# pinellolab/GRAFIMO

Measured on AMD Instinct MI355X. Metric: scored haplotype k-mers/sec, higher is better.
Workload: dtype int32

## Files before the change

### grafimo_amd/csrc/gfm_score_quad.hpp

```cpp
#pragma once

#include "gfm_score_kernels.hpp"
#include "gfm_quad_launch.hpp"

namespace {

typedef unsigned u32x2_t __attribute__((ext_vector_type(2)));
typedef unsigned u32x4_t __attribute__((ext_vector_type(4)));
typedef __attribute__((address_space(3))) const u32x2_t lds_cu32x2;
typedef __attribute__((address_space(3))) const u32x4_t lds_cu32x4;
typedef int i32x4 __attribute__((ext_vector_type(4)));

template <int W, int MM, bool STORE = true>
__global__ void __launch_bounds__(kThreads)
score_quad_kernel(const uint8_t *__restrict__ kmers, long long n, long long row_base, const ScoreArgs<MM> a)
{
    extern __shared__ __attribute__((aligned(16))) unsigned char smem[];
    constexpr int NDW = (W + 3) / 4;
    constexpr int kTabBytes = quad_tab_bytes(W, MM);
    constexpr int CB = kQuadRows * W;
    constexpr int kLoads = (CB + 1023) / 1024;
    constexpr int GP = quad_pitch(W);
    constexpr int PAD = quad_pad(W);
    constexpr int SSTRIDE = quad_strip_stride(W, MM);

    if (lds_offset(smem) != 0u) __builtin_trap();
    const int tid = threadIdx.x;
    const int lane = tid & (kWave - 1);
    const int wave = __builtin_amdgcn_readfirstlane(tid >> 6);
    const int n_waves = (int)(blockDim.x >> 6);
    const int wg_threads = (int)blockDim.x;
    unsigned char *tab = smem;
    unsigned char *stage_base = smem + kTabBytes;
    unsigned *hist[MM];
    {
        unsigned *h = reinterpret_cast<unsigned *>(stage_base + n_waves * SSTRIDE);
#pragma unroll
        for (int m = 0; m < MM; ++m) {
            hist[m] = h;
            if (a.m[m].use_hist) h += a.m[m].nb + 1;
        }
    }

    unsigned char *stage = stage_base + wave * SSTRIDE;
    const unsigned stage_off = (unsigned)(kTabBytes + wave * SSTRIDE);
    const long long nfull = n / kQuadRows;
    const long long cstride = (long long)gridDim.x * n_waves;
    bool vec_store = true;
    const bool through = a.store_through == 1;
    constexpr bool no_store = !STORE;
#pragma unroll
    for (int m = 0; m < MM; ++m) vec_store = vec_store && (reinterpret_cast<uintptr_t>(a.m[m].scores) & 15u) == 0;

    uint4 pre[kQuadDepth][kLoads];
    auto fetch = [&](uint4 (&dst)[kLoads], long long c) {
        const uint8_t *src = kmers + c * (long long)CB + lane * 16;
#pragma unroll
        for (int i = 0; i < kLoads; ++i) {
            if (i * 1024 + 1024 <= CB || i * 1024 + lane * 16 < CB) {
                typedef unsigned u32x4 __attribute__((ext_vector_type(4)));
                const u32x4 t = __builtin_nontemporal_load(reinterpret_cast<const u32x4 *>(src + i * 1024));
                dst[i] = make_uint4(t.x, t.y, t.z, t.w);
            }
        }
    };

    long long *hitq[MM];
    int qn[MM];
    bool select[MM];
#pragma unroll
    for (int m = 0; m < MM; ++m) {
        hitq[m] = reinterpret_cast<long long *>(stage + quad_stage_bytes(W)) + m * kHitQueue;
        qn[m] = 0;
        select[m] = a.m[m].cutoff != GFM_NO_SELECT;
        if (select[m] && blockIdx.x == 0 && tid == 0)
            a.m[m].ctl->snap[a.m[m].slot] = a.m[m].hit_count ? *a.m[m].hit_count : 0ull;
    }

    int p_score[MM][4];
    long long p_crow = -1;
    auto book = [&]() {
        const int k0 = 4 * lane;
#pragma unroll
        for (int m = 0; m < MM; ++m) {
            const MotifArgs &ma = a.m[m];
            if (ma.use_hist) {
#pragma unroll
                for (int j = 0; j < 4; ++j) {
                    const unsigned off = (unsigned)(p_score[m][j] - ma.lo);
                    if (off < (unsigned)ma.nb)
                        atomicAdd(&hist[m][off], 1u);
                    else if (p_score[m][j] == ma.min_val)
                        atomicAdd(&hist[m][ma.nb], 1u);
                    else
                        atomicAdd(&ma.spill[(size_t)(blockIdx.x & (kSpillCopies - 1)) * (size_t)ma.spill_n + (size_t)(p_score[m][j] - ma.spill_lo)], 1u);
                }
            }
            if (select[m]) {
                const int best = max(max(p_score[m][0], p_score[m][1]), max(p_score[m][2], p_score[m][3]));
                if (__builtin_amdgcn_ballot_w64(best >= ma.cutoff)) {
#pragma unroll
                    for (int j = 0; j < 4; ++j)
                        hitq_push(hitq[m], qn[m], p_score[m][j] >= ma.cutoff,
                                  ((row_base + p_crow + k0 + j) << GFM_HIT_SCORE_BITS) | (long long)p_score[m][j], lane,
                                  ma.hit_count, &ma.ctl->mid[ma.slot], ma.hit_rows, ma.hit_cap);
                }
            }
        }
    };

    long long c = (long long)blockIdx.x * n_waves + wave;
#pragma unroll
    for (int d = 0; d < kQuadDepth; ++d)
        if (c + d * cstride < nfull) fetch(pre[d], c + d * cstride);
    if constexpr (MM == 1) {
        for (int i = tid; i < kTabBytes / 2; i += wg_threads) reinterpret_cast<uint16_t *>(tab)[i] = a.m[0].tab[i];
    } else {
        for (int i = tid; i < kTabBytes / 8; i += wg_threads) {
            unsigned long long v = 0;
            if (a.m[0].tab[i] == kPoison) {
                v = 1ull << 57;
            } else {
#pragma unroll
                for (int m = 0; m < MM; ++m) v |= (unsigned long long)a.m[m].tab[i] << (19 * m);
            }
            reinterpret_cast<unsigned long long *>(tab)[i] = v;
        }
    }
#pragma unroll
    for (int m = 0; m < MM; ++m)
        if (a.m[m].use_hist)
            for (int i = tid; i <= a.m[m].nb; i += wg_threads) hist[m][i] = 0u;
    __syncthreads();

    while (c < nfull) {
#pragma unroll
        for (int d = 0; d < kQuadDepth; ++d) {
            if (c >= nfull) break;
            const long long crow = c * kQuadRows;
            if (p_crow >= 0) book();
#pragma unroll
            for (int i = 0; i < kLoads; ++i) {
                const int off = i * 1024 + lane * 16;
                if (i * 1024 + 1024 <= CB || off < CB) {
                    const int dst = PAD ? off + PAD * (off / (4 * W)) : off;
                    *reinterpret_cast<uint4 *>(stage + dst) = pre[d][i];
                }
            }
            if (c + kQuadDepth * cstride < nfull) fetch(pre[d], c + kQuadDepth * cstride);
            __builtin_amdgcn_fence(__ATOMIC_RELEASE, "wavefront");
            __builtin_amdgcn_wave_barrier();

            unsigned w[W + 1];
            {
                const unsigned base = stage_off + (unsigned)(lane * GP);
                if constexpr (W % 2 == 1) {
#pragma unroll
                    for (int t = 0; t < W; ++t) w[t] = ((lds_cu32 *)(uintptr_t)base)[t];
                } else if constexpr (W % 4 == 2) {
#pragma unroll
                    for (int t = 0; t < W / 2; ++t) {
                        const u32x2_t v = ((lds_cu32x2 *)(uintptr_t)base)[t];
                        w[2 * t] = v.x;
                        w[2 * t + 1] = v.y;
                    }
                } else {
#pragma unroll
                    for (int t = 0; t < W / 4; ++t) {
                        const u32x4_t v = ((lds_cu32x4 *)(uintptr_t)base)[t];
                        w[4 * t] = v.x;
                        w[4 * t + 1] = v.y;
                        w[4 * t + 2] = v.z;
                        w[4 * t + 3] = v.w;
                    }
                }
                w[W] = 0u;
            }
            int score[MM][4];
#pragma unroll
            for (int j = 0; j < 4; ++j) {
                const int r = (j * W) & 3;
                bool any_n;
                int acc[MM];
                if constexpr (MM == 1) {
                    int s1 = 0;
#pragma unroll
                    for (int t = 0; t < NDW; ++t) {
                        const int q = (j * W + 4 * t) >> 2;
                        const unsigned x = r ? __builtin_amdgcn_alignbit(w[q + 1], w[q], (unsigned)(8 * r)) : w[q];
                        unsigned y;
                        asm("v_bfi_b32 %0, %1, %2, %3" : "=v"(y) : "s"(0x000E000Eu), "v"(x), "v"(x >> 5));
                        const unsigned e0 = y & 0x7Eu;
                        const unsigned e1 = (y >> 16) & 0x7Eu;
                        s1 += *(lds_cu16 *)(uintptr_t)(e0 + (unsigned)((2 * t) * 128));
                        s1 += *(lds_cu16 *)(uintptr_t)(e1 + (unsigned)((2 * t + 1) * 128));
                    }
                    any_n = (unsigned)s1 >= kPoison;
                    acc[0] = s1;
                } else {
                    unsigned long long s64 = 0;
#pragma unroll
                    for (int t = 0; t < NDW; ++t) {
                        const int q = (j * W + 4 * t) >> 2;
                        const unsigned x = r ? __builtin_amdgcn_alignbit(w[q + 1], w[q], (unsigned)(8 * r)) : w[q];
                        unsigned y;
                        asm("v_bfi_b32 %0, %1, %2, %3" : "=v"(y) : "s"(0x000E000Eu), "v"(x), "v"(x >> 5));
                        const unsigned e0 = (y & 0x7Eu) << 2;
                        const unsigned e1 = ((y >> 16) & 0x7Eu) << 2;
                        s64 += *(lds_cu64 *)(uintptr_t)(e0 + (unsigned)((2 * t) * 512));
                        s64 += *(lds_cu64 *)(uintptr_t)(e1 + (unsigned)((2 * t + 1) * 512));
                    }
                    any_n = (s64 >> 57) != 0;
#pragma unroll
                    for (int m = 0; m < MM; ++m) acc[m] = (int)((s64 >> (19 * m)) & 0x7FFFFull);
                }
#pragma unroll
                for (int m = 0; m < MM; ++m) score[m][j] = any_n ? a.m[m].min_val : acc[m];
            }
            const int k0 = 4 * lane;
#pragma unroll
            for (int m = 0; m < MM; ++m) {
                const __amdgpu_buffer_rsrc_t rs =
                    __builtin_amdgcn_make_buffer_rsrc(a.m[m].scores + crow, 0, kQuadRows * 4, 0x00020000);
                if (no_store) {
                } else if (vec_store) {
                    const u32x4_t out = {(unsigned)score[m][0], (unsigned)score[m][1], (unsigned)score[m][2],
                                         (unsigned)score[m][3]};
                    if (through)
                        __builtin_amdgcn_raw_buffer_store_b128(out, rs, k0 * 4, 0, kStoreThrough);
                    else
                        __builtin_amdgcn_raw_buffer_store_b128(out, rs, k0 * 4, 0, kStoreStream);
                } else {
#pragma unroll
                    for (int j = 0; j < 4; ++j) {
                        if (through)
                            __builtin_amdgcn_raw_buffer_store_b32((unsigned)score[m][j], rs, (k0 + j) * 4, 0, kStoreThrough);
                        else
                            __builtin_amdgcn_raw_buffer_store_b32((unsigned)score[m][j], rs, (k0 + j) * 4, 0, kStoreStream);
                    }
                }
#pragma unroll
                for (int j = 0; j < 4; ++j) p_score[m][j] = score[m][j];
            }
            p_crow = crow;
            __builtin_amdgcn_fence(__ATOMIC_ACQUIRE, "wavefront");
            __builtin_amdgcn_wave_barrier();
            c += cstride;
        }
    }
    if (p_crow >= 0) book();
    if (blockIdx.x == gridDim.x - 1 && wave == n_waves - 1 && nfull * kQuadRows < n) {
        const long long first = nfull * kQuadRows;
        const int count = (int)(n - first);
#pragma unroll 1
        for (int r0 = 0; r0 < count; r0 += kWave) {
            const int k = r0 + lane;
            const bool live = k < count;
            const uint8_t *row = kmers + (first + (live ? k : 0)) * (long long)W;
            unsigned long long s64 = 0;
            bool bad = false;
#pragma unroll 1
            for (int p = 0; p < 2 * NDW; ++p) {
                const unsigned b0 = 2 * p < W ? row[2 * p] : (unsigned)'A';
                const unsigned b1 = 2 * p + 1 < W ? row[2 * p + 1] : (unsigned)'A';
                const unsigned e = p * 64 + ((b0 >> 1) & 7u) + 8u * ((b1 >> 1) & 7u);
                if constexpr (MM == 1) {
                    const unsigned v = reinterpret_cast<const uint16_t *>(tab)[e];
                    bad = bad || v == kPoison;
                    s64 += v;
                } else {
                    s64 += reinterpret_cast<const unsigned long long *>(tab)[e];
                }
            }
            if constexpr (MM > 1) bad = (s64 >> 57) != 0;
#pragma unroll
            for (int m = 0; m < MM; ++m) {
                const MotifArgs &ma = a.m[m];
                const int sc = bad ? ma.min_val : (int)((MM == 1 ? s64 : (s64 >> (19 * m))) & 0x7FFFFull);
                if (live) {
                    if (!no_store) ma.scores[first + k] = sc;
                    if (ma.use_hist) {
                        const unsigned off = (unsigned)(sc - ma.lo);
                        if (off < (unsigned)ma.nb)
                            atomicAdd(&hist[m][off], 1u);
                        else if (sc == ma.min_val)
                            atomicAdd(&hist[m][ma.nb], 1u);
                        else
                            atomicAdd(&ma.spill[(size_t)(blockIdx.x & (kSpillCopies - 1)) * (size_t)ma.spill_n + (size_t)(sc - ma.spill_lo)], 1u);
                    }
                }
                if (select[m])
                    hitq_push(hitq[m], qn[m], live && sc >= ma.cutoff,
                              ((row_base + first + k) << GFM_HIT_SCORE_BITS) | (long long)sc, lane, ma.hit_count,
                              &ma.ctl->mid[ma.slot], ma.hit_rows, ma.hit_cap);
            }
        }
    }

    __syncthreads();
#pragma unroll
    for (int m = 0; m < MM; ++m) {
        const MotifArgs &ma = a.m[m];
        if (select[m]) {
            int *wq_n = reinterpret_cast<int *>(tab) + m * kWavesPerWG;
            if (lane == 0) wq_n[wave] = qn[m];
            __syncthreads();
            int base = 0, tot = 0;
            for (int w2 = 0; w2 < n_waves; ++w2) {
                const int v = wq_n[w2];
                if (w2 < wave) base += v;
                tot += v;
            }
            long long *slab = ma.resid + (size_t)blockIdx.x * kResidPerWG;
            for (int i = lane; i < qn[m]; i += kWave) slab[base + i] = hitq[m][i];
            if (tid == 0) ma.resid_n[blockIdx.x] = tot;
        }
        if (ma.use_hist) {
            unsigned *slab = ma.partials + (size_t)blockIdx.x * (size_t)(ma.nb + 1);
            for (int i = tid; i <= ma.nb; i += wg_threads) slab[i] = hist[m][i];
        }
    }
}

}
```

### grafimo_amd/csrc/gfm_stats_kernels.hpp

```cpp
#pragma once

#include "gfm_common.hpp"

namespace {

struct DpJob {
    long long sm;
    long long cum;
    long long bg;
    int W, L, lo, hi;
    double *buf;
    double *pmf;
    double *ptable;
};

constexpr int kDpThreads = 1024;

__global__ void __launch_bounds__(kDpThreads)
pvalue_dp_kernel(const DpJob *__restrict__ jobs, const int *__restrict__ ints, const double *__restrict__ dbls)
{
    const DpJob job = jobs[blockIdx.x];
    const int W = job.W, L = job.L;
    const int *__restrict__ sm = ints + job.sm;
    const int *__restrict__ cum_lo = ints + job.cum;
    const int *__restrict__ cum_hi = cum_lo + W;
    const double *__restrict__ bg = dbls + job.bg;
    double *__restrict__ pmf_out = job.pmf;
    double *cur = job.buf;
    double *prev = job.buf + L;
    const int tid = threadIdx.x;
    {
        const int l0 = cum_lo[0], h0 = cum_hi[0];
        for (int t = l0 + tid; t <= h0; t += kDpThreads) cur[t] = 0.0;
        __syncthreads();
        if (tid == 0)
            for (int nuc = 0; nuc < 4; ++nuc) {
                const int s = sm[nuc * W];
                cur[s] = __dadd_rn(cur[s], __dmul_rn(1.0, bg[nuc]));
            }
        __syncthreads();
    }
    for (int pos = 1; pos < W; ++pos) {
        double *tmp = cur; cur = prev; prev = tmp;
        const int lp = cum_lo[pos - 1], hp = cum_hi[pos - 1];
        const int lc = cum_lo[pos], hc = cum_hi[pos];
        const int s0 = sm[0 * W + pos], s1 = sm[1 * W + pos], s2 = sm[2 * W + pos],
                  s3 = sm[3 * W + pos];
        const double b0 = bg[0], b1 = bg[1], b2 = bg[2], b3 = bg[3];
        for (int t = lc + tid; t <= hc; t += kDpThreads) {
            double acc = 0.0;
            int idx = t - s0;
            if (idx >= lp && idx <= hp) { const double v = prev[idx]; if (v > 0) acc = __dadd_rn(acc, __dmul_rn(v, b0)); }
            idx = t - s1;
            if (idx >= lp && idx <= hp) { const double v = prev[idx]; if (v > 0) acc = __dadd_rn(acc, __dmul_rn(v, b1)); }
            idx = t - s2;
            if (idx >= lp && idx <= hp) { const double v = prev[idx]; if (v > 0) acc = __dadd_rn(acc, __dmul_rn(v, b2)); }
            idx = t - s3;
            if (idx >= lp && idx <= hp) { const double v = prev[idx]; if (v > 0) acc = __dadd_rn(acc, __dmul_rn(v, b3)); }
            cur[t] = acc;
        }
        __syncthreads();
    }
    const int lf = cum_lo[W - 1], hf = cum_hi[W - 1];
    for (int t = tid; t < L; t += kDpThreads) pmf_out[t] = (t >= lf && t <= hf) ? cur[t] : 0.0;
}

constexpr int kScanThreads = 1024;

__global__ void __launch_bounds__(kScanThreads)
ptable_kernel(const DpJob *__restrict__ jobs)
{
    const DpJob job = jobs[blockIdx.x];
    const double *__restrict__ pmf = job.pmf;
    double *__restrict__ ptable = job.ptable;
    const int L = job.L, lo = job.lo, hi = job.hi;
    __shared__ double carry[kScanThreads];
    __shared__ double tot_s;
    const int tid = threadIdx.x;
    const int nb = hi - lo + 1;
    const int per = (nb + kScanThreads - 1) / kScanThreads;
    const int a = lo + min(tid * per, nb), b = lo + min(tid * per + per, nb);
    double run = 0.0;
    for (int j = b - 1; j >= a; --j) {
        run += pmf[j];
        ptable[j] = run;
    }
    carry[tid] = run;
    __syncthreads();
    if (tid == 0) {
        double c = 0.0;
        for (int t = kScanThreads - 1; t >= 0; --t) {
            const double s = carry[t];
            carry[t] = c;
            c = c + s;
        }
        tot_s = c;
    }
    __syncthreads();
    const double c = carry[tid], tot = tot_s;
    for (int j = a; j < b; ++j) ptable[j] = (c + ptable[j]) / tot;
    for (int j = tid; j < lo; j += kScanThreads) ptable[j] = tot / tot;
    for (int j = hi + 1 + tid; j < L; j += kScanThreads) ptable[j] = 0.0;
}

constexpr int kQThreads = 256;
constexpr int kQStreams = 8;
struct QWork {
    unsigned long long blk_cnt[256];
    double blk_min[256];
    unsigned long long n_rows_N;
};

__device__ inline unsigned long long block_sum_u64(unsigned long long v, unsigned long long *sh)
{
    const int lane = threadIdx.x & 63, wave = threadIdx.x >> 6;
#pragma unroll
    for (int d = 32; d > 0; d >>= 1) v += __shfl_down(v, d);
    if (lane == 0) sh[wave] = v;
    __syncthreads();
    unsigned long long t = 0;
#pragma unroll
    for (int w = 0; w < kQThreads / kWave; ++w) t += sh[w];
    __syncthreads();
    return t;
}

__device__ inline void
q_count_body(const unsigned long long *__restrict__ hist, int L, int lo, int hi, int min_val,
             QWork *__restrict__ ws, int *__restrict__ cutoff_out)
{
    __shared__ unsigned long long sh[kQThreads / kWave];
    const int j = lo + blockIdx.x * kQThreads + threadIdx.x;
    const unsigned long long h = j <= hi ? hist[j] : 0ull;
    const unsigned long long tot = block_sum_u64(h, sh);
    if (threadIdx.x == 0) {
        ws->blk_cnt[blockIdx.x] = tot;
        if (blockIdx.x == 0) {
            const bool n_outside = min_val < lo || min_val > hi;
            ws->n_rows_N = n_outside ? hist[min_val] : 0ull;
            if (cutoff_out) *cutoff_out = L;
        }
    }
}

__device__ inline void
q_raw_body(const unsigned long long *__restrict__ hist, const double *__restrict__ ptable, int lo,
           int hi, QWork *__restrict__ ws, double *__restrict__ raw_out, int nblk)
{
    __shared__ unsigned long long sh[kQThreads / kWave];
    __shared__ double shm[kQThreads / kWave];
    const int tid = threadIdx.x, lane = tid & 63, wave = tid >> 6;
    const int blk = blockIdx.x;
    unsigned long long a = 0, t = 0;
    for (int b = tid; b < nblk; b += kQThreads) {
        const unsigned long long v = ws->blk_cnt[b];
        t += v;
        if (b > blk) a += v;
    }
    const unsigned long long n = block_sum_u64(t, sh) + ws->n_rows_N;
    const unsigned long long above_blocks = block_sum_u64(a, sh);
    const double nd = (double)n;
    const int j = lo + blk * kQThreads + tid;
    const bool ok = j <= hi;
    const unsigned long long h = ok ? hist[j] : 0ull;
    unsigned long long cs = h;
#pragma unroll
    for (int d = 1; d < kWave; d <<= 1) {
        const unsigned long long v = __shfl_down(cs, d);
        if (lane + d < kWave) cs += v;
    }
    if (lane == 0) sh[wave] = cs;
    __syncthreads();
    unsigned long long waves_above = 0;
#pragma unroll
    for (int w = 0; w < kQThreads / kWave; ++w)
        if (w > wave) waves_above += sh[w];
    const unsigned long long c_ge = cs + waves_above + above_blocks;
    const double raw = h ? ptable[j] / ((double)c_ge / nd) : INFINITY;
    if (ok) raw_out[j] = raw;
    double m = raw;
#pragma unroll
    for (int d = 32; d > 0; d >>= 1) m = fmin(m, __shfl_down(m, d));
    if (lane == 0) shm[wave] = m;
    __syncthreads();
    if (tid == 0) {
        double bm = INFINITY;
        for (int w = 0; w < kQThreads / kWave; ++w) bm = fmin(bm, shm[w]);
        ws->blk_min[blk] = bm;
    }
}

__device__ inline void
q_final_body(const unsigned long long *hist, const double *__restrict__ ptable, int L, int lo,
             int hi, int min_val, double threshold, int on_qvalue, const QWork *__restrict__ ws,
             double *qtable, int *__restrict__ cutoff_out, unsigned long long *__restrict__ nrows_out,
             unsigned long long *__restrict__ clear, int nblk)
{
    __shared__ unsigned long long sh[kQThreads / kWave];
    __shared__ double shm[kQThreads / kWave];
    __shared__ int first_s;
    const int tid = threadIdx.x, lane = tid & 63, wave = tid >> 6;
    const int blk = blockIdx.x;
    if (tid == 0) first_s = L;
    unsigned long long t = 0;
    double below = INFINITY, all = INFINITY;
    for (int b = tid; b < nblk; b += kQThreads) {
        t += ws->blk_cnt[b];
        const double v = ws->blk_min[b];
        all = fmin(all, v);
        if (b < blk) below = fmin(below, v);
    }
    const unsigned long long n_rows_N = ws->n_rows_N;
    const unsigned long long n = block_sum_u64(t, sh) + n_rows_N;
    const double nd = (double)n;
#pragma unroll
    for (int d = 32; d > 0; d >>= 1) {
        below = fmin(below, __shfl_down(below, d));
        all = fmin(all, __shfl_down(all, d));
    }
    __shared__ double shb[kQThreads / kWave], sha[kQThreads / kWave];
    if (lane == 0) { shb[wave] = below; sha[wave] = all; }
    __syncthreads();
    below = INFINITY; all = INFINITY;
#pragma unroll
    for (int w = 0; w < kQThreads / kWave; ++w) { below = fmin(below, shb[w]); all = fmin(all, sha[w]); }
    const double base = n_rows_N ? ptable[min_val] / (nd / nd) : INFINITY;
    const int j = lo + blk * kQThreads + tid;
    const bool ok = j <= hi;
    double ms = ok ? qtable[j] : INFINITY;
#pragma unroll
    for (int d = 1; d < kWave; d <<= 1) {
        const double v = __shfl_up(ms, d);
        if (lane >= d) ms = fmin(ms, v);
    }
    if (lane == kWave - 1) shm[wave] = ms;
    __syncthreads();
    double waves_below = INFINITY;
#pragma unroll
    for (int w = 0; w < kQThreads / kWave; ++w)
        if (w < wave) waves_below = fmin(waves_below, shm[w]);
    const double q = fmin(fmin(fmin(ms, waves_below), fmin(below, base)), 1.0);
    if (ok) {
        qtable[j] = q;
        const double val = on_qvalue ? q : ptable[j];
        if (val < threshold) atomicMin(&first_s, j);
        if (clear) clear[j] = 0ull;
    }
    const int gtid = blk * kQThreads + tid, gsz = nblk * kQThreads;
    const double q_above = fmin(fmin(base, all), 1.0);
    for (int jj = gtid; jj < lo; jj += gsz) qtable[jj] = fmin(base, 1.0);
    for (int jj = hi + 1 + gtid; jj < L; jj += gsz) qtable[jj] = q_above;
    __syncthreads();
    if (tid == 0) {
        if (cutoff_out && first_s < L) atomicMin(cutoff_out, first_s);
        if (blk == 0) {
            if (nrows_out) *nrows_out = n;
            const bool n_outside = min_val < lo || min_val > hi;
            if (clear && n_outside) clear[min_val] = 0ull;
        }
    }
}

constexpr int kQJobs = 8;
struct QJob {
    const unsigned long long *hist;
    const double *ptable;
    QWork *ws;
    double *qtable;
    int *cutoff;
    unsigned long long *nrows;
    unsigned long long *clear;
    int L, lo, hi, min_val, nblk;
};
struct QJobs {
    QJob j[kQJobs];
    double threshold;
    int on_qvalue;
};

__global__ void __launch_bounds__(kQThreads) q_count_kernel(const QJobs jobs)
{
    const QJob &q = jobs.j[blockIdx.y];
    if ((int)blockIdx.x >= q.nblk) return;
    q_count_body(q.hist, q.L, q.lo, q.hi, q.min_val, q.ws, q.cutoff);
}

__global__ void __launch_bounds__(kQThreads) q_raw_kernel(const QJobs jobs)
{
    const QJob &q = jobs.j[blockIdx.y];
    if ((int)blockIdx.x >= q.nblk) return;
    q_raw_body(q.hist, q.ptable, q.lo, q.hi, q.ws, q.qtable, q.nblk);
}

__global__ void __launch_bounds__(kQThreads) q_final_kernel(const QJobs jobs)
{
    const QJob &q = jobs.j[blockIdx.y];
    if ((int)blockIdx.x >= q.nblk) return;
    q_final_body(q.hist, q.ptable, q.L, q.lo, q.hi, q.min_val, jobs.threshold, jobs.on_qvalue, q.ws, q.qtable,
                 q.cutoff, q.nrows, q.clear, q.nblk);
}

}
```

### grafimo_amd/csrc/grafimo_hip.hip

```cpp

#include <hip/hip_runtime.h>

#include <algorithm>
#include <atomic>
#include <cmath>
#include <cstdarg>
#include <cstdint>
#include <cstdio>
#include <cstdlib>
#include <cstring>
#include <new>
#include <string>
#include <vector>

#include "grafimo_hip.h"

#define GFM_API extern "C" __attribute__((visibility("default")))

#include "gfm_hit_sort.hpp"
#include "gfm_common.hpp"
#include "gfm_score_kernels.hpp"
#include "gfm_quad_launch.hpp"
#include "gfm_stats_kernels.hpp"

// ... 815 lines not shown
    if (n < 0) return fail(GFM_ERR_INVALID, "negative row count");
    hipStream_t st = static_cast<hipStream_t>(stream);
    hipStream_t tail = tail_stream ? static_cast<hipStream_t>(tail_stream) : st;
    const bool split = tail != st;
    if (n == 0) {
        if ((flags & GFM_FLAG_RESET_HITS) && d_hit_count) {
            if (split) {
                HIP_TRY(hipEventRecord(m->ev_scored[0], st));
                HIP_TRY(hipStreamWaitEvent(tail, m->ev_scored[0], 0));
            }
            HIP_TRY(hipMemsetAsync(d_hit_count, 0, sizeof(uint64_t), tail));
        }
        return GFM_OK;
    }
    if (!d_kmers) return fail(GFM_ERR_INVALID, "NULL device buffer");
    {
        int dev = -1;
        HIP_TRY(hipGetDevice(&dev));
        if (dev != m->device)
            return fail(GFM_ERR_INVALID, "the motif lives on device %d, the current device is %d", m->device, dev);
    }
    if ((reinterpret_cast<uintptr_t>(d_kmers) & 15u) != 0)
        return fail(GFM_ERR_INVALID, "d_kmers must be 16-byte aligned");
    if ((reinterpret_cast<uintptr_t>(d_scores) & 3u) != 0)
        return fail(GFM_ERR_INVALID, "d_scores must be 4-byte aligned");
    if (!d_scores && !d_hist && select_cutoff == GFM_NO_SELECT)
        return fail(GFM_ERR_INVALID, "nothing to do: no scores, no histogram, no selection");
    if (n > (int64_t)kQuadRows * 0x7fffff00ll)
        return fail(GFM_ERR_INVALID, "too many rows for one launch (split the batch)");
    const bool select = select_cutoff != GFM_NO_SELECT;
    if (select && (!d_hit_rows || !d_hit_count))
        return fail(GFM_ERR_INVALID, "selection requested without hit buffers");
    const int use_hist = d_hist ? 1 : 0;
    const long long nchunks = (n + kQuadRows - 1) / kQuadRows;
    const long long want = (nchunks + m->q_waves - 1) / m->q_waves;
    const int avail = split ? std::max(1, m->max_slabs - m->reserve_cus * (m->max_slabs / m->n_cu)) : m->max_slabs;
    int nslabs = (int)std::min<long long>(want, avail);
    if (want > avail) {
        long long best_cap = -1;
        for (int g = avail; g >= std::max(1, avail - avail / 8); --g) {
            const long long per_turn = (long long)g * m->q_waves;
            const long long cap = (nchunks + per_turn - 1) / per_turn * per_turn;
            if (best_cap < 0 || cap < best_cap) { best_cap = cap; nslabs = g; }
        }
#ifdef GFM_LAB
        if (const char *e = std::getenv("GRAFIMO_SCORE_GRID")) {
            const int g = atoi(e);
            if (g >= 1 && g <= m->max_slabs) nslabs = g;
        }
#endif
    }

    const unsigned k = m->call_no++;
    const int ws = (int)(k % (unsigned)kWorkspaces), slot = (int)(k % (unsigned)kCtlSlots);
    const int ws_prev = (int)((k + kWorkspaces - 1) % (unsigned)kWorkspaces);
    const bool reset = (flags & GFM_FLAG_RESET_HITS) != 0;
    const bool same_owner = st == m->last_st && tail == m->last_tail;
    const bool caller_orders = (flags & GFM_FLAG_CALLER_ORDERS_REUSE) && same_owner && m->same_pair_run >= (unsigned)kWorkspaces;
    m->same_pair_run = same_owner ? m->same_pair_run + 1 : 1;
    m->last_st = st;
    m->last_tail = tail;
    if (m->posted_valid[ws] && !caller_orders)
        HIP_TRY(hipStreamWaitEvent(st, m->ev_posted[ws], 0));
    if (split && select && !reset && m->posted_valid[ws_prev])
        HIP_TRY(hipStreamWaitEvent(st, m->ev_posted[ws_prev], 0));
    ScoreArgs<1> args{};
    args.store_through = d_scores ? score_store_through(n, 1) : 2;
    fill_motif_args(args.m[0], m, ws, slot, use_hist, m->hlo, m->hnb, select_cutoff, d_scores,
                    reinterpret_cast<long long *>(d_hit_rows), hit_capacity,
                    reset ? nullptr : reinterpret_cast<unsigned long long *>(d_hit_count));
    hipEvent_t scored = split ? m->ev_scored[ws] : nullptr;
    int rc = dispatch_quad(m->W, 1, m, d_kmers, n, row_base, &args, m->lds_bytes, nslabs, m->q_waves, st, false,
                           split ? &scored : nullptr);
    if (rc) return rc;
    if (split) HIP_TRY(hipStreamWaitEvent(tail, scored, 0));
    m->tail_pending = -1;
    if (split && m->ev_last >= 0 && !m->tev0.empty()) {
        HIP_TRY(hipEventRecord(m->tev0[m->ev_last], tail));
        m->tail_pending = m->ev_last;
    }
    rc = launch_post(m, m->d_partials[ws], nslabs, reinterpret_cast<unsigned long long *>(d_hist),
                     m->hlo, m->hnb, m->d_spill[ws], m->d_resid[ws], m->d_resid_n[ws], select ? nslabs : 0, m->d_ctl, slot,
                     reinterpret_cast<long long *>(d_hit_rows), hit_capacity,
                     reinterpret_cast<unsigned long long *>(d_hit_count), tail);
    if (rc) return rc;
    if (split) {
        HIP_TRY(hipEventRecord(m->ev_posted[ws], tail));
        m->posted_valid[ws] = true;
    } else {
        m->posted_valid[ws] = false;
    }
    return GFM_OK;
}

GFM_API int gfm_score_kmers_multi(const gfm_motif_t *motifs, int n_motifs, const uint8_t *d_kmers,
                                  int64_t n, int32_t *const *d_scores, uint64_t *const *d_hist,
                                  const int32_t *select_cutoffs, int64_t row_base,
                                  int64_t *const *d_hit_rows, const int64_t *hit_capacity,
                                  uint64_t *const *d_hit_count, uint32_t flags, void *stream)
{
    if (!motifs || n_motifs < 1) return fail(GFM_ERR_INVALID, "NULL argument");
    if (n < 0) return fail(GFM_ERR_INVALID, "negative row count");
    hipStream_t st = static_cast<hipStream_t>(stream);
    const bool reset = (flags & GFM_FLAG_RESET_HITS) != 0;
    bool no_scores = d_scores == nullptr;
    if (d_scores) {
        int n_null = 0;
        for (int i = 0; i < n_motifs; ++i) n_null += d_scores[i] ? 0 : 1;
        if (n_null != 0 && n_null != n_motifs) return fail(GFM_ERR_INVALID, "d_scores: every entry or none (scores are stored for all motifs of a call or for none)");
        no_scores = n_null == n_motifs;
    }
    for (int i = 0; i < n_motifs; ++i) {
        if (!motifs[i]) return fail(GFM_ERR_INVALID, "motif %d is NULL", i);
        if (motifs[i]->W != motifs[0]->W)
            return fail(GFM_ERR_INVALID, "motifs of one batched launch must share their width (%d vs %d)",
                        motifs[i]->W, motifs[0]->W);
        for (int j = 0; j < i; ++j)
            if (motifs[j] == motifs[i]) return fail(GFM_ERR_INVALID, "motif %d listed twice", i);
        const bool sel = select_cutoffs && select_cutoffs[i] != GFM_NO_SELECT;
        if (sel && (!d_hit_rows || !d_hit_rows[i] || !d_hit_count || !d_hit_count[i] || !hit_capacity))
            return fail(GFM_ERR_INVALID, "selection requested for motif %d without hit buffers", i);
    }
    if (n == 0) {
        if (reset && d_hit_count)
            for (int i = 0; i < n_motifs; ++i)
                if (d_hit_count[i]) HIP_TRY(hipMemsetAsync(d_hit_count[i], 0, sizeof(uint64_t), st));
        return GFM_OK;
    }
    if (!d_kmers) return fail(GFM_ERR_INVALID, "NULL device buffer");
    if ((reinterpret_cast<uintptr_t>(d_kmers) & 15u) != 0)
        return fail(GFM_ERR_INVALID, "d_kmers must be 16-byte aligned");
    if (n > (int64_t)kQuadRows * 0x7fffff00ll)
        return fail(GFM_ERR_INVALID, "too many rows for one launch (split the batch)");
    for (int i = 0; i < n_motifs && !no_scores; ++i)
        if ((reinterpret_cast<uintptr_t>(d_scores[i]) & 3u) != 0)
            return fail(GFM_ERR_INVALID, "d_scores[%d] must be 4-byte aligned", i);
    const int W = motifs[0]->W;
    const long long nchunks = (n + kQuadRows - 1) / kQuadRows;

    int i = 0;
    while (i < n_motifs) {
        int mm = 0, waves = kWavesPerWG, nb_lds[3] = {0, 0, 0};
        int win_lo[3] = {0, 0, 0}, win_nb[3] = {0, 0, 0};
        bool with_hist[3];
        for (int k = 0; k < 3; ++k) with_hist[k] = i + k < n_motifs && d_hist && d_hist[i + k];
        if (!plan_group(motifs + i, n_motifs - i, with_hist, &mm, &waves, win_lo, win_nb))
            return fail(GFM_ERR_INVALID, "no LDS left for a histogram window at width %d", W);
        for (int k = 0; k < mm; ++k) {
            if (win_nb[k] > motifs[i + k]->part_nb)
                return fail(GFM_ERR_INVALID, "internal error: histogram window larger than the workspace");
            nb_lds[k] = (d_hist && d_hist[i + k]) ? win_nb[k] + 1 : 0;
        }
        size_t lds = quad_fixed_lds(W, waves, mm);
        for (int k = 0; k < mm; ++k) lds += sizeof(unsigned) * (size_t)nb_lds[k];
        const long long want = (nchunks + waves - 1) / waves;
        int nslabs = (int)std::min<long long>(want, motifs[i]->max_slabs);
        for (int k = 1; k < mm; ++k) nslabs = std::min(nslabs, motifs[i + k]->max_slabs);
        int ws[3], slot[3], uh[3];
        ScoreArgs<1> a1{};
        ScoreArgs<2> a2{};
        ScoreArgs<3> a3{};
        a1.store_through = a2.store_through = a3.store_through = no_scores ? 2 : score_store_through(n, mm);
        for (int k = 0; k < mm; ++k) {
            gfm_motif *mo = motifs[i + k];
            const unsigned c = mo->call_no++;
            mo->same_pair_run = 0;
            mo->last_st = mo->last_tail = nullptr;
            ws[k] = (int)(c % (unsigned)kWorkspaces);
            slot[k] = (int)(c % (unsigned)kCtlSlots);
            mo->posted_valid[ws[k]] = false;
            uh[k] = (d_hist && d_hist[i + k]) ? 1 : 0;
            const int cut = select_cutoffs ? select_cutoffs[i + k] : GFM_NO_SELECT;
            const bool sel = cut != GFM_NO_SELECT;
            MotifArgs &dst = mm == 1 ? a1.m[k] : (mm == 2 ? a2.m[k] : a3.m[k]);
            fill_motif_args(dst, mo, ws[k], slot[k], uh[k], win_lo[k], win_nb[k], cut, no_scores ? nullptr : d_scores[i + k],
                            sel ? reinterpret_cast<long long *>(d_hit_rows[i + k]) : nullptr,
                            sel ? hit_capacity[i + k] : 0,
                            (sel && !reset) ? reinterpret_cast<const unsigned long long *>(d_hit_count[i + k])
                                            : nullptr);
        }
        const void *args = mm == 1 ? static_cast<const void *>(&a1) : (mm == 2 ? static_cast<const void *>(&a2) : &a3);
        int rc = dispatch_quad(W, mm, motifs[i], d_kmers, n, row_base, args, lds, nslabs, waves, st, false);
        if (rc) return rc;
        PostJob posts[kPostJobs];
        for (int k = 0; k < mm; ++k) {
            gfm_motif *mo = motifs[i + k];
            const int cut = select_cutoffs ? select_cutoffs[i + k] : GFM_NO_SELECT;
            const bool sel = cut != GFM_NO_SELECT;
            posts[k] = post_job(mo, mo->d_partials[ws[k]], nslabs,
                                uh[k] ? reinterpret_cast<unsigned long long *>(d_hist[i + k]) : nullptr,
                                win_lo[k], win_nb[k], mo->d_spill[ws[k]], mo->d_resid[ws[k]], mo->d_resid_n[ws[k]],
                                sel ? nslabs : 0, mo->d_ctl, slot[k],
                                sel ? reinterpret_cast<long long *>(d_hit_rows[i + k]) : nullptr,
                                sel ? hit_capacity[i + k] : 0,
                                sel ? reinterpret_cast<unsigned long long *>(d_hit_count[i + k]) : nullptr);
        }
        rc = launch_posts(posts, mm, st);
        if (rc) return rc;
        i += mm;
    }
    return GFM_OK;
}

GFM_API int gfm_score_kmers_multi_plan(const gfm_motif_t *motifs, int n_motifs, const int32_t *with_hist,
                                       int32_t *group_size_out, int32_t *waves_out)
{
    if (!motifs || n_motifs < 1) return fail(GFM_ERR_INVALID, "NULL argument");
    for (int i = 0; i < n_motifs; ++i) {
        if (!motifs[i]) return fail(GFM_ERR_INVALID, "motif %d is NULL", i);
        if (motifs[i]->W != motifs[0]->W)
            return fail(GFM_ERR_INVALID, "motifs of one batched launch must share their width (%d vs %d)",
                        motifs[i]->W, motifs[0]->W);
    }
    int i = 0;
    while (i < n_motifs) {
        int mm = 0, waves = 0, win_lo[3], win_nb[3];
        bool wh[3];
        for (int k = 0; k < 3; ++k) wh[k] = i + k < n_motifs && (!with_hist || with_hist[i + k]);
        if (!plan_group(motifs + i, n_motifs - i, wh, &mm, &waves, win_lo, win_nb))
            return fail(GFM_ERR_INVALID, "no LDS left for a histogram window at width %d", motifs[0]->W);
        for (int k = 0; k < mm; ++k) {
            if (group_size_out) group_size_out[i + k] = mm;
            if (waves_out) waves_out[i + k] = waves;
        }
        i += mm;
    }
    return GFM_OK;
}

GFM_API int gfm_profile_enable(gfm_motif_t m, int slots, int every)
{
    if (!m || slots < 0 || every < 1) return fail(GFM_ERR_INVALID, "bad argument");
    m->ev_every = every;
    m->ev_calls = 0;
    for (auto e : m->ev0) (void)hipEventDestroy(e);
    for (auto e : m->ev1) (void)hipEventDestroy(e);
    for (auto e : m->tev0) (void)hipEventDestroy(e);
    for (auto e : m->tev1) (void)hipEventDestroy(e);
    m->ev0.clear();
    m->ev1.clear();
    m->tev0.clear();
    m->tev1.clear();
    m->tail_order.clear();
    m->ev_next = m->ev_used = 0;
    m->ev_last = m->tail_pending = -1;
    for (int i = 0; i < slots; ++i) {
        hipEvent_t a, b, c, d;
        HIP_TRY(hipEventCreate(&a));
        HIP_TRY(hipEventCreate(&b));
        HIP_TRY(hipEventCreate(&c));
        HIP_TRY(hipEventCreate(&d));
        m->ev0.push_back(a);
        m->ev1.push_back(b);
        m->tev0.push_back(c);
        m->tev1.push_back(d);
    }
    return GFM_OK;
}

GFM_API int gfm_profile_mark_tail(gfm_motif_t m, void *stream)
{
    if (!m) return fail(GFM_ERR_INVALID, "motif is NULL");
    if (m->tail_pending < 0) return GFM_OK;
    HIP_TRY(hipEventRecord(m->tev1[m->tail_pending], static_cast<hipStream_t>(stream)));
    if ((int)m->tail_order.size() < (int)m->tev0.size()) m->tail_order.push_back(m->tail_pending);
    m->tail_pending = -1;
    return GFM_OK;
}

GFM_API int gfm_profile_read_tail(gfm_motif_t m, float *h_ms, int capacity, int *n_out)
{
    if (!m || !n_out || (!h_ms && capacity)) return fail(GFM_ERR_INVALID, "NULL argument");
    const int used = std::min((int)m->tail_order.size(), capacity);
    for (int i = 0; i < used; ++i) {
        const int slot = m->tail_order[(size_t)i];
        HIP_TRY(hipEventSynchronize(m->tev1[slot]));
        HIP_TRY(hipEventElapsedTime(&h_ms[i], m->tev0[slot], m->tev1[slot]));
    }
    *n_out = used;
    m->tail_order.clear();
    return GFM_OK;
}

GFM_API int gfm_profile_read(gfm_motif_t m, float *h_ms, int capacity, int *n_out)
{
    if (!m || !n_out || (!h_ms && capacity)) return fail(GFM_ERR_INVALID, "NULL argument");
    const int slots = (int)m->ev0.size();
    const int used = std::min(m->ev_used, capacity);
    for (int i = 0; i < used; ++i) {
        const int slot = ((m->ev_next - m->ev_used + i) % slots + slots) % slots;
        HIP_TRY(hipEventSynchronize(m->ev1[slot]));
        HIP_TRY(hipEventElapsedTime(&h_ms[i], m->ev0[slot], m->ev1[slot]));
    }
    *n_out = used;
    m->ev_used = 0;
    return GFM_OK;
}

namespace {
int launch_qtables(const gfm_motif_t *motifs, int count, uint64_t *const *d_hist, double threshold, int on_qvalue,
                   double *const *d_qtable, int32_t *const *d_cutoff, uint64_t *const *d_nrows, uint32_t flags,
                   hipStream_t st)
{
    QJobs jobs{};
    jobs.threshold = threshold;
    jobs.on_qvalue = on_qvalue;
    int max_blk = 0;
    for (int k = 0; k < count; ++k) {
        gfm_motif *m = motifs[k];
        QJob &q = jobs.j[k];
        q.hist = reinterpret_cast<const unsigned long long *>(d_hist[k]);
        q.ptable = m->d_ptable;
        int qs = 0;
        while (qs < m->q_streams_used && m->q_stream[qs] != st) ++qs;
        if (qs == m->q_streams_used) {
            if (qs < kQStreams) {
                ++m->q_streams_used;
            } else {
                qs = 0;
                for (int c = 1; c < kQStreams; ++c)
                    if (m->q_last_use[c] < m->q_last_use[qs]) qs = c;
            }
            m->q_stream[qs] = st;
        }
        m->q_last_use[qs] = ++m->q_calls;
        q.ws = m->d_qwork + qs;
        q.qtable = (d_qtable && d_qtable[k]) ? d_qtable[k] : m->d_qscratch + (size_t)qs * (size_t)m->L;
        q.cutoff = d_cutoff ? d_cutoff[k] : nullptr;
        q.nrows = d_nrows ? reinterpret_cast<unsigned long long *>(d_nrows[k]) : nullptr;
        q.clear = (flags & GFM_FLAG_CLEAR_HIST) ? reinterpret_cast<unsigned long long *>(d_hist[k]) : nullptr;
        q.L = m->L; q.lo = m->lo; q.hi = m->hi; q.min_val = m->min_val;
        q.nblk = (m->nb + kQThreads - 1) / kQThreads;
        max_blk = std::max(max_blk, q.nblk);
    }
    const dim3 grid((unsigned)max_blk, (unsigned)count);
    hipLaunchKernelGGL(q_count_kernel, grid, dim3(kQThreads), 0, st, jobs);
    hipLaunchKernelGGL(q_raw_kernel, grid, dim3(kQThreads), 0, st, jobs);
    hipLaunchKernelGGL(q_final_kernel, grid, dim3(kQThreads), 0, st, jobs);
    HIP_TRY(hipGetLastError());
    return GFM_OK;
}
}

GFM_API int gfm_qvalue_table(gfm_motif_t m, uint64_t *d_hist, double threshold, int on_qvalue,
                             double *d_qtable, int32_t *d_cutoff, uint64_t *d_nrows, uint32_t flags,
                             void *stream)
{
    if (!m || !d_hist) return fail(GFM_ERR_INVALID, "NULL argument");
    return launch_qtables(&m, 1, &d_hist, threshold, on_qvalue, &d_qtable, &d_cutoff, &d_nrows, flags,
                          static_cast<hipStream_t>(stream));
}

GFM_API int gfm_qvalue_table_multi(const gfm_motif_t *motifs, int n_motifs, uint64_t *const *d_hist,
                                   double threshold, int on_qvalue, double *const *d_qtable,
                                   int32_t *const *d_cutoff, uint64_t *const *d_nrows, uint32_t flags, void *stream)
{
    if (!motifs || n_motifs < 1 || !d_hist) return fail(GFM_ERR_INVALID, "NULL argument");
    for (int i = 0; i < n_motifs; ++i) {
        if (!motifs[i] || !d_hist[i]) return fail(GFM_ERR_INVALID, "motif or histogram %d is NULL", i);
        for (int j = 0; j < i; ++j)
            if (motifs[j] == motifs[i]) return fail(GFM_ERR_INVALID, "motif %d listed twice", i);
    }
    for (int i = 0; i < n_motifs; i += kQJobs) {
        const int count = std::min(kQJobs, n_motifs - i);
        const int rc = launch_qtables(motifs + i, count, d_hist + i, threshold, on_qvalue,
                                      d_qtable ? d_qtable + i : nullptr, d_cutoff ? d_cutoff + i : nullptr,
                                      d_nrows ? d_nrows + i : nullptr, flags, static_cast<hipStream_t>(stream));
        if (rc) return rc;
    }
    return GFM_OK;
}

namespace {
int order_selection(gfm_motif *m, hipStream_t st, bool before)
{
    hipStreamCaptureStatus cap = hipStreamCaptureStatusNone;
    if (hipStreamIsCapturing(st, &cap) != hipSuccess) { (void)hipGetLastError(); cap = hipStreamCaptureStatusNone; }
    if (cap != hipStreamCaptureStatusNone) return GFM_OK;
    if (before) {
        if (m->sel_valid && m->sel_last_stream != st) HIP_TRY(hipStreamWaitEvent(st, m->ev_selected, 0));
    } else {
        HIP_TRY(hipEventRecord(m->ev_selected, st));
        m->sel_last_stream = st;
        m->sel_valid = true;
    }
    return GFM_OK;
}
}

GFM_API int gfm_select_hits(gfm_motif_t m, const int32_t *d_scores, int64_t n, const int32_t *d_cutoff,
                            int64_t row_base, int64_t *d_hit_rows, int64_t hit_capacity,
                            uint64_t *d_hit_count, uint32_t flags, void *stream)
{
    if (!m) return fail(GFM_ERR_INVALID, "motif is NULL");
    if (n < 0) return fail(GFM_ERR_INVALID, "negative row count");
    if (n == 0) {
        if ((flags & GFM_FLAG_RESET_HITS) && d_hit_count)
            HIP_TRY(hipMemsetAsync(d_hit_count, 0, sizeof(uint64_t), static_cast<hipStream_t>(stream)));
        return GFM_OK;
    }
    if (!d_scores || !d_cutoff || !d_hit_rows || !d_hit_count)
        return fail(GFM_ERR_INVALID, "NULL device buffer");
    if ((reinterpret_cast<uintptr_t>(d_scores) & 15u) != 0)
        return fail(GFM_ERR_INVALID, "d_scores must be 16-byte aligned");
    hipStream_t st = static_cast<hipStream_t>(stream);
    const long long n4 = (n + 3) >> 2;
    long long blocks = (n4 + kSelThreads - 1) / kSelThreads;
    blocks = std::max<long long>(1, std::min<long long>(blocks, m->sel_slabs));
    const int slot = (int)(m->sel_call_no++ % (unsigned)kCtlSlots);
    {
        const int rc0 = order_selection(m, st, true);
        if (rc0) return rc0;
    }
    hipLaunchKernelGGL(select_hits_kernel, dim3((unsigned)blocks), dim3(kSelThreads), 0, st, d_scores,
                       (long long)n, d_cutoff, (long long)row_base,
                       reinterpret_cast<long long *>(d_hit_rows), (long long)hit_capacity,
                       (flags & GFM_FLAG_RESET_HITS)
                           ? nullptr
                           : reinterpret_cast<const unsigned long long *>(d_hit_count),
                       m->d_sel_ctl, slot, m->d_sel_resid, m->d_sel_resid_n,
                       static_cast<const unsigned long long *>(nullptr), 0ll);
    HIP_TRY(hipGetLastError());
    const int rc = launch_post(m, nullptr, 0, nullptr, 0, 0, nullptr, m->d_sel_resid, m->d_sel_resid_n, (int)blocks,
                               m->d_sel_ctl, slot, reinterpret_cast<long long *>(d_hit_rows), hit_capacity,
                               reinterpret_cast<unsigned long long *>(d_hit_count), st);
    return rc ? rc : order_selection(m, st, false);
}

GFM_API int gfm_select_hits_from(gfm_motif_t m, const int32_t *d_scores, int64_t n, const int32_t *d_cutoff,
                                 int64_t row_base, const int64_t *d_cand_rows, int64_t cand_capacity,
                                 const uint64_t *d_cand_count, int64_t *d_hit_rows, int64_t hit_capacity,
                                 uint64_t *d_hit_count, void *stream)
{
    if (!m) return fail(GFM_ERR_INVALID, "motif is NULL");
    if (n < 0 || cand_capacity < 0) return fail(GFM_ERR_INVALID, "negative row count or capacity");
    hipStream_t st = static_cast<hipStream_t>(stream);
    if (n == 0) {
        if (d_hit_count) HIP_TRY(hipMemsetAsync(d_hit_count, 0, sizeof(uint64_t), st));
        return GFM_OK;
    }
    if (!d_cutoff || !d_cand_rows || !d_cand_count || !d_hit_rows || !d_hit_count)
        return fail(GFM_ERR_INVALID, "NULL device buffer");
    if (d_cand_rows == d_hit_rows || reinterpret_cast<const void *>(d_cand_count) == d_hit_count)
        return fail(GFM_ERR_INVALID, "the candidate list and the hit list must be different buffers");
    if ((reinterpret_cast<uintptr_t>(d_scores) & 15u) != 0)
        return fail(GFM_ERR_INVALID, "d_scores must be 16-byte aligned");
    {
        const int rc0 = order_selection(m, st, true);
        if (rc0) return rc0;
    }
    {
        const long long blocks = std::max<long long>(1, (cand_capacity + kFilterPerBlock - 1) / kFilterPerBlock);
        HIP_TRY(hipMemsetAsync(d_hit_count, 0, sizeof(uint64_t), st));
        hipLaunchKernelGGL(filter_hits_kernel, dim3((unsigned)blocks), dim3(kSelThreads), 0, st,
                           reinterpret_cast<const long long *>(d_cand_rows),
                           reinterpret_cast<const unsigned long long *>(d_cand_count), (long long)cand_capacity, d_cutoff,
                           reinterpret_cast<long long *>(d_hit_rows), (long long)hit_capacity,
                           reinterpret_cast<unsigned long long *>(d_hit_count));
        HIP_TRY(hipGetLastError());
    }
    if (!d_scores) return order_selection(m, st, false);
    const long long n4 = (n + 3) >> 2;
    long long blocks = (n4 + kSelThreads - 1) / kSelThreads;
    blocks = std::max<long long>(1, std::min<long long>(blocks, m->sel_slabs));
    const int slot = (int)(m->sel_call_no++ % (unsigned)kCtlSlots);
    hipLaunchKernelGGL(select_hits_kernel, dim3((unsigned)blocks), dim3(kSelThreads), 0, st, d_scores,
                       (long long)n, d_cutoff, (long long)row_base, reinterpret_cast<long long *>(d_hit_rows),
                       (long long)hit_capacity, reinterpret_cast<const unsigned long long *>(d_hit_count),
                       m->d_sel_ctl, slot, m->d_sel_resid, m->d_sel_resid_n,
                       reinterpret_cast<const unsigned long long *>(d_cand_count), (long long)cand_capacity);
    HIP_TRY(hipGetLastError());
    const int rc = launch_post(m, nullptr, 0, nullptr, 0, 0, nullptr, m->d_sel_resid, m->d_sel_resid_n, (int)blocks,
                               m->d_sel_ctl, slot, reinterpret_cast<long long *>(d_hit_rows), hit_capacity,
                               reinterpret_cast<unsigned long long *>(d_hit_count), st);
    return rc ? rc : order_selection(m, st, false);
}

GFM_API int gfm_scan_host(gfm_motif_t m, const uint8_t *h_kmers, int64_t n, double threshold,
                          int on_qvalue, int want_qvalues, int64_t capacity, int64_t *h_rows,
                          int32_t *h_scores, double *h_logodds, double *h_pvalue, double *h_qvalue,
                          int64_t *n_hits)
{
    if (!m || !n_hits) return fail(GFM_ERR_INVALID, "NULL argument");
    *n_hits = 0;
    if (n < 0 || capacity < 0) return fail(GFM_ERR_INVALID, "negative size");
    if (!(threshold > 0 && threshold <= 1)) return fail(GFM_ERR_INVALID, "threshold must be in (0, 1]");
    if (on_qvalue && !want_qvalues) return fail(GFM_ERR_INVALID, "q-value threshold without q-values");
    if (n == 0) return GFM_OK;
    if (!h_kmers) return fail(GFM_ERR_INVALID, "h_kmers is NULL");

    const size_t kbytes = (size_t)n * (size_t)m->W;
    uint8_t *d_kmers = nullptr;
    int *d_scores = nullptr, *d_cutoff = nullptr;
    unsigned long long *d_hist = nullptr, *d_count = nullptr;
    long long *d_rows = nullptr;
    double *d_q = nullptr;
    hipStream_t st = nullptr;
    int rc = GFM_OK;
    std::vector<long long> rows;
    std::vector<double> q;
    unsigned long long cnt = 0;
    const long long cap = std::max<long long>(capacity, 1);
    const bool need_hist = want_qvalues != 0;

#define SCAN_TRY(expr)                                                                  \
    do {                                                                                \
        hipError_t e_ = (expr);                                                         \
        if (e_ != hipSuccess) {                                                         \
            rc = fail(GFM_ERR_HIP, "%s failed: %s", #expr, hipGetErrorString(e_));      \
            goto done;                                                                  \
        }                                                                               \
    } while (0)
#define SCAN_RC(expr)            \
    do {                         \
        rc = (expr);             \
        if (rc) goto done;       \
    } while (0)

    SCAN_TRY(hipStreamCreate(&st));
    SCAN_TRY(hipMalloc(&d_kmers, kbytes + 16));
    SCAN_TRY(hipMalloc(&d_scores, sizeof(int) * (size_t)n));
    SCAN_TRY(hipMalloc(&d_rows, sizeof(long long) * (size_t)cap));
    SCAN_TRY(hipMalloc(&d_count, sizeof(unsigned long long)));
    SCAN_TRY(hipMalloc(&d_cutoff, sizeof(int)));
    SCAN_TRY(hipMemsetAsync(d_count, 0, sizeof(unsigned long long), st));
    if (need_hist) {
        SCAN_TRY(hipMalloc(&d_hist, sizeof(unsigned long long) * (size_t)m->L));
        SCAN_TRY(hipMalloc(&d_q, sizeof(double) * (size_t)m->L));
        SCAN_TRY(hipMemsetAsync(d_hist, 0, sizeof(unsigned long long) * (size_t)m->L, st));
    }
    SCAN_TRY(hipMemcpyAsync(d_kmers, h_kmers, kbytes, hipMemcpyHostToDevice, st));
    if (!on_qvalue) {
        int32_t cutoff = 0;
        SCAN_RC(gfm_motif_pvalue_cutoff(m, threshold, &cutoff));
        SCAN_RC(gfm_score_kmers(m, d_kmers, n, d_scores, reinterpret_cast<uint64_t *>(d_hist), cutoff,
                                0, reinterpret_cast<int64_t *>(d_rows), cap,
                                reinterpret_cast<uint64_t *>(d_count), GFM_FLAG_RESET_HITS, st, nullptr));
        if (need_hist)
            SCAN_RC(gfm_qvalue_table(m, reinterpret_cast<uint64_t *>(d_hist), threshold, 0, d_q,
                                     nullptr, nullptr, 0, st));
    } else {
        SCAN_RC(gfm_score_kmers(m, d_kmers, n, d_scores, reinterpret_cast<uint64_t *>(d_hist),
                                GFM_NO_SELECT, 0, nullptr, 0, nullptr, 0, st, nullptr));
        SCAN_RC(gfm_qvalue_table(m, reinterpret_cast<uint64_t *>(d_hist), threshold, 1, d_q, d_cutoff,
                                 nullptr, 0, st));
        SCAN_RC(gfm_select_hits(m, d_scores, n, d_cutoff, 0, reinterpret_cast<int64_t *>(d_rows), cap,
                                reinterpret_cast<uint64_t *>(d_count), GFM_FLAG_RESET_HITS, st));
    }
    SCAN_TRY(hipMemcpyAsync(&cnt, d_count, sizeof cnt, hipMemcpyDeviceToHost, st));
    SCAN_TRY(hipStreamSynchronize(st));
    *n_hits = (int64_t)cnt;
    if ((long long)cnt > capacity) {
        rc = fail(GFM_ERR_OVERFLOW, "%llu hits exceed the capacity of %lld rows", cnt, (long long)capacity);
        goto done;
    }
    if (cnt) {
        rows.resize(cnt);
        SCAN_TRY(hipMemcpyAsync(rows.data(), d_rows, sizeof(long long) * cnt, hipMemcpyDeviceToHost, st));
        if (need_hist) {
            q.resize(m->L);
            SCAN_TRY(hipMemcpyAsync(q.data(), d_q, sizeof(double) * (size_t)m->L, hipMemcpyDeviceToHost, st));
        }
        SCAN_TRY(hipStreamSynchronize(st));
        gfm_hit_sort::sort_packed(reinterpret_cast<int64_t *>(rows.data()), rows.size(), GFM_HIT_SCORE_BITS);
        for (size_t i = 0; i < cnt; ++i) {
            const int s = (int)(rows[i] & ((1ll << GFM_HIT_SCORE_BITS) - 1));
            if (h_rows) h_rows[i] = rows[i] >> GFM_HIT_SCORE_BITS;
            if (h_scores) h_scores[i] = s;
            if (h_logodds) h_logodds[i] = ((double)s / (double)m->scale) + ((double)m->W * m->offset);
            if (h_pvalue) h_pvalue[i] = m->h_ptable[s];
            if (h_qvalue && need_hist) h_qvalue[i] = q[s];
        }
    }
done:
#undef SCAN_TRY
#undef SCAN_RC
    if (d_kmers) (void)hipFree(d_kmers);
    if (d_scores) (void)hipFree(d_scores);
    if (d_rows) (void)hipFree(d_rows);
    if (d_count) (void)hipFree(d_count);
    if (d_cutoff) (void)hipFree(d_cutoff);
    if (d_hist) (void)hipFree(d_hist);
    if (d_q) (void)hipFree(d_q);
    if (st) (void)hipStreamDestroy(st);
    return rc;
}
```

Before: 219.5 billion.

## Fuse q-value table into single-block kernel and use LDS atomics for histogram

Adds a single-workgroup q_table_kernel that computes counts, suffix sums, raw q-values and their running minimum in one launch for a single motif with a small bin range, replacing three separate kernel launches. The score kernel's shared-memory histogram updates are merged into one branch and issued as explicit LDS-addressed relaxed workgroup-scope atomics. The aim is to cut launch overhead in the q-value step and branch/address overhead in the scoring hot loop. The fused kernel duplicates logic from the three-kernel path and could diverge from it numerically.

Result: faster. 225.3 billion (median of 6 runs) (+2.6%).

```diff
diff --git a/grafimo_amd/csrc/gfm_score_quad.hpp b/grafimo_amd/csrc/gfm_score_quad.hpp
--- a/grafimo_amd/csrc/gfm_score_quad.hpp
+++ b/grafimo_amd/csrc/gfm_score_quad.hpp
@@ -10,6 +10,12 @@
 typedef __attribute__((address_space(3))) const u32x2_t lds_cu32x2;
 typedef __attribute__((address_space(3))) const u32x4_t lds_cu32x4;
 typedef int i32x4 __attribute__((ext_vector_type(4)));
+
+__device__ inline void lds_hist_add(unsigned window, unsigned bin)
+{
+    typedef __attribute__((address_space(3))) unsigned lds_u32;
+    __hip_atomic_fetch_add((lds_u32 *)(uintptr_t)(window + 4u * bin), 1u, __ATOMIC_RELAXED, __HIP_MEMORY_SCOPE_WORKGROUP);
+}
 
 template <int W, int MM, bool STORE = true>
 __global__ void __launch_bounds__(kThreads)
@@ -33,11 +39,13 @@
     unsigned char *tab = smem;
     unsigned char *stage_base = smem + kTabBytes;
     unsigned *hist[MM];
+    unsigned hist_off[MM];
     {
         unsigned *h = reinterpret_cast<unsigned *>(stage_base + n_waves * SSTRIDE);
 #pragma unroll
         for (int m = 0; m < MM; ++m) {
             hist[m] = h;
+            hist_off[m] = lds_offset(h);
             if (a.m[m].use_hist) h += a.m[m].nb + 1;
         }
     }
@@ -88,10 +96,8 @@
 #pragma unroll
                 for (int j = 0; j < 4; ++j) {
                     const unsigned off = (unsigned)(p_score[m][j] - ma.lo);
-                    if (off < (unsigned)ma.nb)
-                        atomicAdd(&hist[m][off], 1u);
-                    else if (p_score[m][j] == ma.min_val)
-                        atomicAdd(&hist[m][ma.nb], 1u);
+                    if (off < (unsigned)ma.nb || p_score[m][j] == ma.min_val)
+                        lds_hist_add(hist_off[m], min(off, (unsigned)ma.nb));
                     else
                         atomicAdd(&ma.spill[(size_t)(blockIdx.x & (kSpillCopies - 1)) * (size_t)ma.spill_n + (size_t)(p_score[m][j] - ma.spill_lo)], 1u);
                 }
@@ -281,10 +287,8 @@
                     if (!no_store) ma.scores[first + k] = sc;
                     if (ma.use_hist) {
                         const unsigned off = (unsigned)(sc - ma.lo);
-                        if (off < (unsigned)ma.nb)
-                            atomicAdd(&hist[m][off], 1u);
-                        else if (sc == ma.min_val)
-                            atomicAdd(&hist[m][ma.nb], 1u);
+                        if (off < (unsigned)ma.nb || sc == ma.min_val)
+                            lds_hist_add(hist_off[m], min(off, (unsigned)ma.nb));
                         else
                             atomicAdd(&ma.spill[(size_t)(blockIdx.x & (kSpillCopies - 1)) * (size_t)ma.spill_n + (size_t)(sc - ma.spill_lo)], 1u);
                     }
diff --git a/grafimo_amd/csrc/gfm_stats_kernels.hpp b/grafimo_amd/csrc/gfm_stats_kernels.hpp
--- a/grafimo_amd/csrc/gfm_stats_kernels.hpp
+++ b/grafimo_amd/csrc/gfm_stats_kernels.hpp
@@ -300,4 +300,114 @@
                  q.cutoff, q.nrows, q.clear, q.nblk);
 }
 
-}
+constexpr int kQ1Threads = 512;
+constexpr int kQ1K = 16;
+constexpr int kQ1Bins = kQ1Threads * kQ1K;
+constexpr int kQ1Waves = kQ1Threads / kWave;
+
+__global__ void __launch_bounds__(kQ1Threads) q_table_kernel(const QJobs jobs)
+{
+    const QJob &q = jobs.j[blockIdx.x];
+    const unsigned long long *hist = q.hist;
+    const double *__restrict__ ptable = q.ptable;
+    double *qtable = q.qtable;
+    unsigned long long *clear = q.clear;
+    const int L = q.L, lo = q.lo, hi = q.hi, min_val = q.min_val;
+    __shared__ unsigned long long sh_cnt[kQ1Waves];
+    __shared__ double sh_min[kQ1Waves];
+    __shared__ unsigned long long sh_n_rows_N;
+    __shared__ int first_s;
+    const int tid = threadIdx.x, lane = tid & (kWave - 1), wave = tid >> 6;
+    const int j0 = lo + tid * kQ1K;
+    const bool n_outside = min_val < lo || min_val > hi;
+    if (tid == 0) {
+        sh_n_rows_N = n_outside ? hist[min_val] : 0ull;
+        first_s = L;
+    }
+    unsigned long long c[kQ1K];
+    double p[kQ1K];
+    unsigned occ = 0;
+#pragma unroll
+    for (int k = 0; k < kQ1K; ++k) c[k] = j0 + k <= hi ? hist[j0 + k] : 0ull;
+#pragma unroll
+    for (int k = 0; k < kQ1K; ++k) p[k] = j0 + k <= hi ? ptable[j0 + k] : 0.0;
+    const double p_min_val = ptable[min_val];
+    unsigned long long run = 0;
+#pragma unroll
+    for (int k = kQ1K - 1; k >= 0; --k) {
+        occ |= (c[k] != 0ull ? 1u : 0u) << k;
+        run += c[k];
+        c[k] = run;
+    }
+    unsigned long long cs = run;
+#pragma unroll
+    for (int d = 1; d < kWave; d <<= 1) {
+        const unsigned long long v = __shfl_down(cs, d);
+        if (lane + d < kWave) cs += v;
+    }
+    if (lane == 0) sh_cnt[wave] = cs;
+    __syncthreads();
+    unsigned long long above = cs - run, total = 0;
+#pragma unroll
+    for (int w = 0; w < kQ1Waves; ++w) {
+        const unsigned long long v = sh_cnt[w];
+        total += v;
+        if (w > wave) above += v;
+    }
+    const unsigned long long n_rows_N = sh_n_rows_N;
+    const unsigned long long n = total + n_rows_N;
+    const double nd = (double)n;
+    double r[kQ1K];
+    double m = INFINITY;
+    unsigned p_below = 0;
+#pragma unroll
+    for (int k = 0; k < kQ1K; ++k) {
+        double raw = INFINITY;
+        if ((occ >> k) & 1u) raw = p[k] / ((double)(c[k] + above) / nd);
+        p_below |= (p[k] < jobs.threshold ? 1u : 0u) << k;
+        m = fmin(m, raw);
+        r[k] = m;
+    }
+    double ms = m;
+#pragma unroll
+    for (int d = 1; d < kWave; d <<= 1) {
+        const double v = __shfl_up(ms, d);
+        if (lane >= d) ms = fmin(ms, v);
+    }
+    if (lane == kWave - 1) sh_min[wave] = ms;
+    double below = __shfl_up(ms, 1);
+    if (lane == 0) below = INFINITY;
+    __syncthreads();
+    double all = INFINITY;
+#pragma unroll
+    for (int w = 0; w < kQ1Waves; ++w) {
+        const double v = sh_min[w];
+        all = fmin(all, v);
+        if (w < wave) below = fmin(below, v);
+    }
+    const double base = n_rows_N ? p_min_val / (nd / nd) : INFINITY;
+    below = fmin(below, base);
+    int first = L;
+#pragma unroll
+    for (int k = kQ1K - 1; k >= 0; --k) {
+        const int j = j0 + k;
+        if (j <= hi) {
+            const double qv = fmin(fmin(r[k], below), 1.0);
+            qtable[j] = qv;
+            if (jobs.on_qvalue ? qv < jobs.threshold : ((p_below >> k) & 1u) != 0) first = j;
+            if (clear) clear[j] = 0ull;
+        }
+    }
+    if (first < L) atomicMin(&first_s, first);
+    const double q_above = fmin(fmin(base, all), 1.0);
+    for (int jj = tid; jj < lo; jj += kQ1Threads) qtable[jj] = fmin(base, 1.0);
+    for (int jj = hi + 1 + tid; jj < L; jj += kQ1Threads) qtable[jj] = q_above;
+    __syncthreads();
+    if (tid == 0) {
+        if (q.cutoff) *q.cutoff = first_s;
+        if (q.nrows) *q.nrows = n;
+        if (clear && n_outside) clear[min_val] = 0ull;
+    }
+}
+
+}
diff --git a/grafimo_amd/csrc/grafimo_hip.hip b/grafimo_amd/csrc/grafimo_hip.hip
--- a/grafimo_amd/csrc/grafimo_hip.hip
+++ b/grafimo_amd/csrc/grafimo_hip.hip
@@ -1141,13 +1141,14 @@
                    double *const *d_qtable, int32_t *const *d_cutoff, uint64_t *const *d_nrows, uint32_t flags,
                    hipStream_t st)
 {
-    QJobs jobs{};
-    jobs.threshold = threshold;
-    jobs.on_qvalue = on_qvalue;
-    int max_blk = 0;
+    QJobs one{}, three{};
+    one.threshold = three.threshold = threshold;
+    one.on_qvalue = three.on_qvalue = on_qvalue;
+    int n_one = 0, n_three = 0, max_blk = 0;
     for (int k = 0; k < count; ++k) {
         gfm_motif *m = motifs[k];
-        QJob &q = jobs.j[k];
+        const bool narrow = count == 1 && m->nb <= kQ1Bins;
+        QJob &q = narrow ? one.j[n_one++] : three.j[n_three++];
         q.hist = reinterpret_cast<const unsigned long long *>(d_hist[k]);
         q.ptable = m->d_ptable;
         int qs = 0;
@@ -1170,12 +1171,15 @@
         q.clear = (flags & GFM_FLAG_CLEAR_HIST) ? reinterpret_cast<unsigned long long *>(d_hist[k]) : nullptr;
         q.L = m->L; q.lo = m->lo; q.hi = m->hi; q.min_val = m->min_val;
         q.nblk = (m->nb + kQThreads - 1) / kQThreads;
-        max_blk = std::max(max_blk, q.nblk);
-    }
-    const dim3 grid((unsigned)max_blk, (unsigned)count);
-    hipLaunchKernelGGL(q_count_kernel, grid, dim3(kQThreads), 0, st, jobs);
-    hipLaunchKernelGGL(q_raw_kernel, grid, dim3(kQThreads), 0, st, jobs);
-    hipLaunchKernelGGL(q_final_kernel, grid, dim3(kQThreads), 0, st, jobs);
+        if (!narrow) max_blk = std::max(max_blk, q.nblk);
+    }
+    if (n_one) hipLaunchKernelGGL(q_table_kernel, dim3((unsigned)n_one), dim3(kQ1Threads), 0, st, one);
+    if (n_three) {
+        const dim3 grid((unsigned)max_blk, (unsigned)n_three);
+        hipLaunchKernelGGL(q_count_kernel, grid, dim3(kQThreads), 0, st, three);
+        hipLaunchKernelGGL(q_raw_kernel, grid, dim3(kQThreads), 0, st, three);
+        hipLaunchKernelGGL(q_final_kernel, grid, dim3(kQThreads), 0, st, three);
+    }
     HIP_TRY(hipGetLastError());
     return GFM_OK;
 }
```
